# smallflyingpig/speech-to-image-translation-without-text

Hardware: AMD Instinct MI355X
Metric: StackGAN-v2 3-stage G+D train-step images/sec at 256px (higher is better)
Workload: dtype f32

## Files before the change

include/s2i_hip.h:

```cpp
#ifndef S2I_HIP_H
#define S2I_HIP_H

#include <stddef.h>
#include <stdint.h>

#ifdef __cplusplus
extern "C" {
#endif

#define S2I_ABI_VERSION 4

#define S2I_CONV_K1      0
#define S2I_CONV_K3S1    1
#define S2I_CONV_K4S2    2
#define S2I_TCONV_K4S2   3

#define S2I_CONV_1D      4

#define S2I_ACT_NONE     0
#define S2I_ACT_GLU      1
#define S2I_ACT_LRELU    2
#define S2I_ACT_TANH     3
#define S2I_ACT_RELU     4

#define S2I_DT_F32       0
#define S2I_DT_BF16      1

#define S2I_PACK_PLAIN   0
#define S2I_PACK_UPFOLD  1

const char* s2i_last_error(void);
int  s2i_version(void);
int  s2i_set_tuning(const char* key, int value);
int  s2i_get_tuning(const char* key, int* value);
int  s2i_check_device(void);

typedef struct s2i_conv_desc {
  int kind;
  int B, H, W;
  int Cx;
  int Cc;
  int N;
  int wmode;
  int flip;
  int wR;
  int ldw;
  int act;
  int stats;
  int ldy;
  int groups;
  int nosplit;
  int kw, stride, pad;
  int tile_rows;
  int in_act;
  int in_groups;
} s2i_conv_desc;

size_t s2i_conv_workspace_bytes(const s2i_conv_desc* d);
int    s2i_conv_stat_parts(const s2i_conv_desc* d);
int s2i_conv_forward(const s2i_conv_desc* d, const float* x, const float* cvec, const float* w,
                     const float* bias, float* y, float* part, void* ws, size_t ws_bytes,
                     void* stream);

int s2i_conv_forward_cls(const s2i_conv_desc* d, const float* x, const float* cvec, const float* w,
                         const float* bias, const float* cls_bias, float* y, float* part, void* ws,
                         size_t ws_bytes, void* stream);

int s2i_conv_forward_in(const s2i_conv_desc* d, const float* x_raw, const float* in_coef, const float* w, float* y,
                        float* part, void* ws, size_t ws_bytes, void* stream);

int s2i_cvec_bias_table(const float* cvec, const float* packed, int B, int Cc, int Ip, int Op, int N,
                        float* table, void* ws , size_t ws_bytes, void* stream);
size_t s2i_border_sums_workspace_bytes(int B, int H, int W, int C);
int s2i_tap_sums(const float* dy, int B, int H, int W, int C, float* tapsum, void* ws, size_t ws_bytes,
                 void* stream);
int s2i_cvec_grads(const float* cvec, const float* packed, const float* tapsum, int B, int Cc, int Ip,
                   int Op, int N, int O, int I_total, float* dc, float* dw_oihw, int accumulate,
                   void* stream);

typedef struct s2i_wgrad_desc {
  int kind;
  int B, H, W;
  int Ca;
  int Cc;
  int N;
  int ldg;
  int swap;
  int fold;
  int O, I, KH, KW;
  int accumulate;
  int i_off;
  int I_total;
  int a_act;
  int a_groups;
} s2i_wgrad_desc;

size_t s2i_wgrad_workspace_bytes(const s2i_wgrad_desc* d);
int s2i_conv_wgrad(const s2i_wgrad_desc* d, const float* a, const float* cvec, const float* g,
                   float* grad_oihw, void* ws, size_t ws_bytes, void* stream);

int s2i_conv_wgrad_in_eligible(const s2i_wgrad_desc* d);
int s2i_conv_wgrad_in(const s2i_wgrad_desc* d, const float* a_raw, const float* a_coef, const float* g,
                      float* grad_oihw, void* ws, size_t ws_bytes, void* stream);


int s2i_conv_split_eligible(const s2i_conv_desc* d);
int s2i_conv_forward_split(const s2i_conv_desc* d, const float* x, const float* cvec,
                           const unsigned short* wsplit, int planes, int np, int kp, const float* bias,
                           const float* cls_bias, float* y, float* part, void* ws, size_t ws_bytes,
                           void* stream);
size_t s2i_wgrad_workspace_bytes_split(const s2i_wgrad_desc* d, int planes);
int s2i_conv_wgrad_split(const s2i_wgrad_desc* d, int planes, const float* a, const float* cvec,
                         const float* g, float* grad_oihw, void* ws, size_t ws_bytes, void* stream);
int s2i_split_packed_weight(const float* packed, int T, int R, int C, int planes, unsigned short* out_rc,
                            unsigned short* out_cr, void* stream);


int    s2i_conv_bf16_eligible(const s2i_conv_desc* d);
size_t s2i_conv_bf16_workspace_bytes(const s2i_conv_desc* d);
int    s2i_conv_bf16_stat_parts(const s2i_conv_desc* d);
size_t s2i_conv_bf16_weight_elems(const s2i_conv_desc* d);
int    s2i_conv_bf16_weight_layout(const s2i_conv_desc* d);
int s2i_pack_conv_weight_bf16(const s2i_conv_desc* d, const float* packed, int R, int C, unsigned short* out,
                              void* stream);
typedef struct s2i_pack16_item {
  const float* P;
  unsigned short* out;
  int R, C, kind, flip, transpose, T, nphase, Nn, Npad, Kk, CK, gx, gy, block0;
} s2i_pack16_item;
int s2i_pack16_item_fill(const s2i_conv_desc* d, const float* packed, int R, int C, unsigned short* out,
                         s2i_pack16_item* item);
int s2i_pack_conv_weights_bf16_batched(const s2i_pack16_item* items_dev, int n, int total_blocks, void* stream);
int s2i_conv_forward_bf16(const s2i_conv_desc* d, const unsigned short* x, const unsigned short* w,
                          const float* cls_bias, unsigned short* y, float* part, void* ws, size_t ws_bytes,
                          void* stream);
int s2i_conv_forward_dt(const s2i_conv_desc* d, const void* x, int x_dtype, const float* cvec, const float* w,
                        const float* bias, const float* cls_bias, void* y, int y_dtype, float* part, void* ws,
                        size_t ws_bytes, void* stream);
size_t s2i_wgrad_workspace_bytes_dt(const s2i_wgrad_desc* d, int a_dtype, int g_dtype);
int s2i_conv_wgrad_dt(const s2i_wgrad_desc* d, const void* a, int a_dtype, const float* cvec, const void* g,
                      int g_dtype, float* grad_oihw, void* ws, size_t ws_bytes, void* stream);
int s2i_bn_act_forward_dt(int dtype, const void* y, long long M, int groups, int C, const float* coef4, int act,
                          const void* residual, void* out, void* stream);
int s2i_bn_act_bwd_reduce_dt(int dtype, const void* y, const void* dout, int lddout, long long M, int groups, int C,
                             const float* coef4, int act, float* part, int nparts, void* stream);
int s2i_bn_act_bwd_apply_dt(int dtype, const void* y, const void* dout, int lddout, long long M, int groups, int C,
                            const float* coef4, const float* red2, int act, void* dy, void* stream);
int s2i_act_backward_dt(int dtype, const void* out, const void* dout, int lddout, long long M, int C, int act,
                        void* dy, void* stream);
// ... 162 lines not shown
```

speech_to_image_translation_without_text_amd/_lib.py:

```python
import ctypes
import os

import torch

_HERE = os.path.dirname(os.path.abspath(__file__))
LIB_PATH = os.path.join(_HERE, "libs2i_hip.so")

CONV_K1, CONV_K3S1, CONV_K4S2, TCONV_K4S2, CONV_1D = 0, 1, 2, 3, 4
ACT_NONE, ACT_GLU, ACT_LRELU, ACT_TANH, ACT_RELU = 0, 1, 2, 3, 4
PACK_PLAIN, PACK_UPFOLD = 0, 1
DT_F32, DT_BF16 = 0, 1
POOL_MAX3S2, POOL_AVG3S1, POOL_GLOBAL = 0, 1, 2
POOL_THEN_LRN, LRN_THEN_POOL = 0, 1
LOGMEL_BFT, LOGMEL_NHWC = 0, 1
LOGMEL_TILE_FRAMES = 64
ABI_VERSION = 4

c_int, c_float, c_void_p, c_size_t, c_ll = (ctypes.c_int, ctypes.c_float, ctypes.c_void_p,
                                            ctypes.c_size_t, ctypes.c_longlong)


class ConvDesc(ctypes.Structure):
    _fields_ = [(n, c_int) for n in ("kind", "B", "H", "W", "Cx", "Cc", "N", "wmode", "flip", "wR",
                                     "ldw", "act", "stats", "ldy", "groups", "nosplit", "kw", "stride", "pad",
                                     "tile_rows", "in_act", "in_groups")]


class Conv2dDesc(ctypes.Structure):
    _fields_ = [(n, c_int) for n in ("B", "H", "W", "C", "ldx", "N", "kh", "kw", "sh", "sw", "ph", "pw", "Ho", "Wo",
                                     "ldy", "coff", "relu", "tile")]


class WgradDesc(ctypes.Structure):
    _fields_ = [(n, c_int) for n in ("kind", "B", "H", "W", "Ca", "Cc", "N", "ldg", "swap", "fold",
                                     "O", "I", "KH", "KW", "accumulate", "i_off", "I_total", "a_act", "a_groups")]


class PackItem(ctypes.Structure):
    _fields_ = [("w", c_void_p), ("packed", c_void_p)] + [(n, c_int) for n in ("O", "I", "KH", "KW", "Ip", "mode", "gx",
                                                                               "block0")]


class Pack16Item(ctypes.Structure):
    _fields_ = [("P", c_void_p), ("out", c_void_p)] + [(n, c_int) for n in (
        "R", "C", "kind", "flip", "transpose", "T", "nphase", "Nn", "Npad", "Kk", "CK", "gx", "gy", "block0")]


P = c_void_p
_SIGNATURES = {
    "s2i_last_error": (ctypes.c_char_p, []),
    "s2i_version": (c_int, []),
    "s2i_check_device": (c_int, []),
    "s2i_set_tuning": (c_int, [ctypes.c_char_p, c_int]),
    "s2i_get_tuning": (c_int, [ctypes.c_char_p, ctypes.POINTER(c_int)]),
    "s2i_conv_workspace_bytes": (c_size_t, [ctypes.POINTER(ConvDesc)]),
    "s2i_conv_stat_parts": (c_int, [ctypes.POINTER(ConvDesc)]),
    "s2i_conv_forward": (c_int, [ctypes.POINTER(ConvDesc), P, P, P, P, P, P, P, c_size_t, P]),
    "s2i_conv_forward_cls": (c_int, [ctypes.POINTER(ConvDesc), P, P, P, P, P, P, P, P, c_size_t, P]),
    "s2i_conv_forward_in": (c_int, [ctypes.POINTER(ConvDesc), P, P, P, P, P, P, c_size_t, P]),
    "s2i_conv_wgrad_in_eligible": (c_int, [ctypes.POINTER(WgradDesc)]),
    "s2i_conv_wgrad_in": (c_int, [ctypes.POINTER(WgradDesc), P, P, P, P, P, c_size_t, P]),
    "s2i_conv_split_eligible": (c_int, [ctypes.POINTER(ConvDesc)]),
    "s2i_conv_forward_split": (c_int, [ctypes.POINTER(ConvDesc), P, P, P, c_int, c_int, c_int, P, P, P, P, P, c_size_t, P]),
    "s2i_split_packed_weight": (c_int, [P, c_int, c_int, c_int, c_int, P, P, P]),
    "s2i_wgrad_workspace_bytes_split": (c_size_t, [ctypes.POINTER(WgradDesc), c_int]),
    "s2i_conv_wgrad_split": (c_int, [ctypes.POINTER(WgradDesc), c_int, P, P, P, P, P, c_size_t, P]),
    "s2i_conv_bf16_eligible": (c_int, [ctypes.POINTER(ConvDesc)]),
    "s2i_conv_bf16_workspace_bytes": (c_size_t, [ctypes.POINTER(ConvDesc)]),
    "s2i_conv_bf16_stat_parts": (c_int, [ctypes.POINTER(ConvDesc)]),
    "s2i_conv_bf16_weight_elems": (c_size_t, [ctypes.POINTER(ConvDesc)]),
    "s2i_conv_bf16_weight_layout": (c_int, [ctypes.POINTER(ConvDesc)]),
    "s2i_pack16_item_fill": (c_int, [ctypes.POINTER(ConvDesc), P, c_int, c_int, P, ctypes.POINTER(Pack16Item)]),
    "s2i_pack_conv_weights_bf16_batched": (c_int, [P, c_int, c_int, P]),
    "s2i_pack_conv_weight_bf16": (c_int, [ctypes.POINTER(ConvDesc), P, c_int, c_int, P, P]),
    "s2i_conv_forward_bf16": (c_int, [ctypes.POINTER(ConvDesc), P, P, P, P, P, P, c_size_t, P]),
    "s2i_conv_forward_dt": (c_int, [ctypes.POINTER(ConvDesc), P, c_int, P, P, P, P, P, c_int, P, P, c_size_t, P]),
    "s2i_wgrad_workspace_bytes_dt": (c_size_t, [ctypes.POINTER(WgradDesc), c_int, c_int]),
    "s2i_conv_wgrad_dt": (c_int, [ctypes.POINTER(WgradDesc), P, c_int, P, P, c_int, P, P, c_size_t, P]),
    "s2i_bn_act_forward_dt": (c_int, [c_int, P, c_ll, c_int, c_int, P, c_int, P, P, P]),
    "s2i_bn_act_bwd_reduce_dt": (c_int, [c_int, P, P, c_int, c_ll, c_int, c_int, P, c_int, P, c_int, P]),
    "s2i_bn_act_bwd_apply_dt": (c_int, [c_int, P, P, c_int, c_ll, c_int, c_int, P, P, c_int, P, P]),
    "s2i_act_backward_dt": (c_int, [c_int, P, P, c_int, c_ll, c_int, c_int, P, P]),
    "s2i_nchw_to_nhwc_dt": (c_int, [c_int, P, P, c_int, c_int, c_int, c_int, c_int, P]),
    "s2i_nhwc_to_nchw_dt": (c_int, [c_int, P, c_int, P, c_int, c_int, c_int, c_int, P]),
    "s2i_spatial_sum_dt": (c_int, [c_int, P, c_int, c_int, c_int, c_int, P, P, c_size_t, P]),
    "s2i_tap_sums_dt": (c_int, [c_int, P, c_int, c_int, c_int, c_int, P, P, c_size_t, P]),
    "s2i_cast": (c_int, [P, c_int, P, c_int, c_ll, P]),
    "s2i_cvec_bias_table": (c_int, [P, P, c_int, c_int, c_int, c_int, c_int, P, P, c_size_t, P]),
    "s2i_border_sums_workspace_bytes": (c_size_t, [c_int, c_int, c_int, c_int]),
    "s2i_tap_sums": (c_int, [P, c_int, c_int, c_int, c_int, P, P, c_size_t, P]),
    "s2i_cvec_grads": (c_int, [P, P, P, c_int, c_int, c_int, c_int, c_int, c_int, c_int, P, P, c_int, P]),
    "s2i_wgrad_workspace_bytes": (c_size_t, [ctypes.POINTER(WgradDesc)]),
    "s2i_conv_wgrad": (c_int, [ctypes.POINTER(WgradDesc), P, P, P, P, P, c_size_t, P]),
    "s2i_pack_conv_weight": (c_int, [P, P, c_int, c_int, c_int, c_int, c_int, c_int, P]),
    "s2i_pack_conv_weights_batched": (c_int, [P, c_int, c_int, c_int, P]),
    "s2i_bn_finalize": (c_int, [P, c_int, c_int, c_int, c_ll, P, P, P, P, P, c_float, c_float, P, P]),
    "s2i_bn_eval_coeffs": (c_int, [c_int, P, P, P, P, c_float, P, P]),
    "s2i_bn_act_forward": (c_int, [P, c_ll, c_int, c_int, P, c_int, P, P, P]),
    "s2i_colstats": (c_int, [P, c_ll, c_int, c_int, P, c_int, P]),
    "s2i_bn_act_bwd_reduce": (c_int, [P, P, c_int, c_ll, c_int, c_int, P, c_int, P, c_int, P]),
    "s2i_bn_bwd_finalize": (c_int, [P, c_int, c_int, c_int, c_ll, P, P, c_int, P, P]),
    "s2i_bn_act_bwd_apply": (c_int, [P, P, c_int, c_ll, c_int, c_int, P, P, c_int, P, P]),
    "s2i_act_backward": (c_int, [P, P, c_int, c_ll, c_int, c_int, P, P]),
    "s2i_glu_forward": (c_int, [P, c_ll, c_int, P, P]),
    "s2i_glu_backward": (c_int, [P, P, c_ll, c_int, P, P]),
    "s2i_nchw_to_nhwc": (c_int, [P, P, c_int, c_int, c_int, c_int, c_int, P]),
    "s2i_nhwc_to_nchw": (c_int, [P, c_int, P, c_int, c_int, c_int, c_int, P]),
    "s2i_image_to_u8": (c_int, [P, c_int, P, c_ll, P]),
    "s2i_u8_to_image": (c_int, [P, P, c_int, c_int, c_int, P]),
    "s2i_image_batch": (c_int, [P, c_ll, P, P, c_int, P, c_int, c_int, c_int, P, P, P, P, P, P]),
    "s2i_spatial_sum": (c_int, [P, c_int, c_int, c_int, c_int, P, P, c_size_t, P]),
    "s2i_spatial_sum_workspace_bytes": (c_size_t, [c_int, c_int, c_int]),
    "s2i_reparam_forward": (c_int, [P, P, c_int, c_int, P, P]),
    "s2i_reparam_backward": (c_int, [P, P, P, P, P, c_int, c_int, P, P]),
    "s2i_kl_forward": (c_int, [P, c_int, P, c_int, c_int, c_int, P, P]),
    "s2i_kl_backward": (c_int, [P, c_int, P, c_int, c_int, c_int, P, P, P, P]),
    "s2i_logit_forward": (c_int, [P, P, P, c_int, c_int, P, P]),
    "s2i_logit_backward": (c_int, [P, P, P, P, c_int, c_int, P, c_int, P, P, c_int, P]),
    "s2i_bce_forward": (c_int, [P, c_float, c_int, c_float, P, c_int, P]),
    "s2i_bce_backward": (c_int, [P, c_float, c_int, c_float, P, P, P]),
    "s2i_bce_multi_forward": (c_int, [P, P, P, c_int, c_int, c_int, P, P]),
    "s2i_bce_multi_backward": (c_int, [P, P, P, c_int, c_int, c_int, P, P, P]),
    "s2i_cal_loss": (c_int, [P, P, c_int, c_int, P, c_int, P, P]),
    "s2i_maxpool_w3s2": (c_int, [P, c_int, c_int, c_int, c_int, P, P]),
    "s2i_lstm_cell": (c_int, [P, c_int, P, P, c_int, c_int, c_int, c_int, c_int, P, P, P, c_int, P]),
    "s2i_lstm_step": (c_int, [P, c_int, P, P, P, c_int, c_int, c_int, c_int, c_int, P, P, P, P, c_int, P]),
    "s2i_time_mean": (c_int, [P, c_int, c_int, c_int, P, P]),
    "s2i_adam_step": (c_int, [P, P, P, P, c_ll, c_float, c_float, c_float, c_float, c_int, P, c_float, P]),
    "s2i_increment": (c_int, [P, P]),
    "s2i_ema_update": (c_int, [P, P, c_ll, c_float, P]),
    "s2i_scale_dev": (c_int, [P, P, c_ll, P, P]),
    "s2i_axpby": (c_int, [P, P, c_ll, c_float, c_float, P]),
    "s2i_plan_create": (c_int, [P, ctypes.POINTER(P), ctypes.POINTER(c_int)]),
    "s2i_plan_replay": (c_int, [P, P]),
    "s2i_plan_destroy": (c_int, [P]),
    "s2i_conv2d_plan": (c_int, [ctypes.POINTER(Conv2dDesc)]),
    "s2i_conv2d_weight_elems": (c_size_t, [ctypes.POINTER(Conv2dDesc)]),
    "s2i_conv2d_forward": (c_int, [ctypes.POINTER(Conv2dDesc), P, P, P, P, P]),
    "s2i_pool2d": (c_int, [c_int, P, c_int, c_int, c_int, c_int, c_int, P, c_int, c_int, P]),
    "s2i_inception_prep": (c_int, [P, c_int, c_int, c_int, c_ll, c_ll, c_ll, c_ll, P, c_int, c_int, P]),
    "s2i_softmax_rows": (c_int, [P, c_int, c_int, c_int, P, c_int, P]),
# ... 96 lines not shown
```

speech_to_image_translation_without_text_amd/csrc/s2i_common.h:

```cpp
#pragma once
#include <hip/hip_runtime.h>
#include <stdio.h>
#include <stdarg.h>
#include "../../include/s2i_hip.h"

typedef float f32x16 __attribute__((ext_vector_type(16)));
typedef float f32x4 __attribute__((ext_vector_type(4)));

void s2i_set_error(const char* fmt, ...);

#define S2I_FAIL(...)            \
  do {                           \
    s2i_set_error(__VA_ARGS__);  \
    return 1;                    \
  } while (0)

#define S2I_REQUIRE(cond, ...)   \
  do {                           \
    if (!(cond)) S2I_FAIL(__VA_ARGS__); \
  } while (0)

#define S2I_LAUNCH_CHECK(name)                                          \
  do {                                                                  \
    hipError_t e__ = hipGetLastError();                                 \
    if (e__ != hipSuccess) S2I_FAIL("%s: launch failed: %s", name, hipGetErrorString(e__)); \
  } while (0)

static inline int s2i_ilog2(int v) {
  int l = 0;
  while ((1 << l) < v) ++l;
  return l;
}
static inline bool s2i_is_pow2(int v) { return v > 0 && (v & (v - 1)) == 0; }
static inline int s2i_cdiv(long long a, long long b) { return (int)((a + b - 1) / b); }

enum {
  S2I_TUNE_FWD_BM = 0,
  S2I_TUNE_FWD_MIN_CPS,
  S2I_TUNE_B16_V2,
  S2I_TUNE_B16_PERSIST,
  S2I_TUNE_FINALIZE_THREADS,
  S2I_TUNE_B16_DBG,
  S2I_TUNE_WGRAD16_BM,
  S2I_TUNE_WGRAD_BM,
  S2I_TUNE_COUNT
};
int s2i_tune(int key, int def);
```

speech_to_image_translation_without_text_amd/csrc/s2i_conv.hip:

```cpp
#include "s2i_igemm.h"

namespace {

static int fwd_splitk(long long blocks, int nchunks, int nosplit, int min_cps) {
  int splitk = 1;
  if (blocks < 512 && nchunks >= 16 && !nosplit) {
    splitk = (int)(768 / blocks);
    if (splitk > nchunks / min_cps) splitk = nchunks / min_cps;
    if (splitk > 64) splitk = 64;
    if (splitk < 1) splitk = 1;
  }
  return splitk;
}

int plan_fwd(const s2i_conv_desc* d, FwdPlan* pl) {
  S2I_REQUIRE(d->B > 0 && d->H > 0 && d->W > 0 && d->N > 0, "conv: non-positive extent");
  S2I_REQUIRE(d->Cx >= 0 && d->Cc >= 0 && (d->Cx % 4) == 0 && (d->Cc % 4) == 0 && d->Cx + d->Cc > 0,
              "conv: channel counts must be multiples of 4 (Cx=%d Cc=%d)", d->Cx, d->Cc);
  S2I_REQUIRE(s2i_is_pow2(d->H) && s2i_is_pow2(d->W), "conv: spatial extents must be powers of two");
  pl->Ca = d->Cx + d->Cc;
  pl->nphases = 1;
  switch (d->kind) {
    case S2I_CONV_K1: pl->T = 1; pl->Ho = d->H; pl->Wo = d->W; break;
    case S2I_CONV_K3S1: pl->T = 9; pl->Ho = d->H; pl->Wo = d->W; break;
    case S2I_CONV_K4S2:
      S2I_REQUIRE(d->H >= 2 && d->W >= 2, "conv k4s2: extent < 2");
      pl->T = 16; pl->Ho = d->H / 2; pl->Wo = d->W / 2; break;
    case S2I_TCONV_K4S2: pl->T = 4; pl->Ho = d->H; pl->Wo = d->W; pl->nphases = 4; break;
    case S2I_CONV_1D:
      S2I_REQUIRE(d->kw >= 1 && d->kw <= 31 && d->stride >= 1 && d->pad >= 0, "conv1d: bad kw/stride/pad");
      S2I_REQUIRE(d->wmode == 0 && !d->flip, "conv1d: forward only");
      pl->T = d->kw; pl->Ho = d->H; pl->Wo = (d->W + 2 * d->pad - d->kw) / d->stride + 1;
      S2I_REQUIRE(pl->Wo >= 1 && s2i_is_pow2(pl->Wo), "conv1d: output width %d is not a power of two", pl->Wo);
      break;
    default: S2I_FAIL("conv: unknown kind %d", d->kind);
  }
  const long long M = (long long)d->B * pl->Ho * pl->Wo;
  S2I_REQUIRE(M * 4 < (1ll << 31), "conv: too many rows");
  pl->M = (int)M;
  pl->Mrows = M * pl->nphases;
  pl->K = pl->T * pl->Ca;
  if (d->wmode == 0) {
    S2I_REQUIRE(d->wR >= pl->Ca, "conv: wR (%d) smaller than the gathered channels (%d)", d->wR, pl->Ca);
    S2I_REQUIRE(d->ldw >= d->N && d->ldw % 4 == 0, "conv: ldw %d too small for N %d", d->ldw, d->N);
  } else {
    S2I_REQUIRE(d->wR >= d->N, "conv(T): wR (%d) < N (%d)", d->wR, d->N);
    S2I_REQUIRE(d->ldw >= pl->Ca, "conv(T): ldw (%d) < gathered channels (%d)", d->ldw, pl->Ca);
  }
  S2I_REQUIRE(d->ldy >= d->N, "conv: ldy < N");
  S2I_REQUIRE(!(d->stats && (d->act != S2I_ACT_NONE)), "conv: stats epilogue needs act NONE");
  if (d->stats && d->groups > 1) {
    S2I_REQUIRE(d->kind != S2I_TCONV_K4S2 && (M % d->groups) == 0 &&
                    (((M / d->groups) % 128) == 0 || (d->N > 64 && ((M / d->groups) % 96) == 0 && d->tile_rows != 128)),
                "conv: %lld rows do not split into %d BatchNorm groups of whole row tiles", M, d->groups);
    S2I_REQUIRE((d->N % 4) == 0, "conv: grouped statistics need N %% 4 == 0");
  }
  pl->tile = d->N > 64 ? 0 : (d->N > 32 ? 1 : 2);
  const int BN = pl->tile == 0 ? 128 : (pl->tile == 1 ? 64 : 32);
  pl->gridN = s2i_cdiv(d->N, BN);
  pl->nchunks = s2i_cdiv(pl->K, 32);
  const int forced_bm = d->tile_rows ? d->tile_rows : s2i_tune(S2I_TUNE_FWD_BM, 0);
  S2I_REQUIRE(forced_bm == 0 || forced_bm == 96 || forced_bm == 128, "conv: tile_rows must be 0, 96 or 128");
  const int min_cps = s2i_tune(S2I_TUNE_FWD_MIN_CPS, 4);
  static const int cand_bm[2] = {128, 96};
  double best = 1e300;
  int best_bm = 128, best_split = 1;
  for (int c = 0; c < 2; ++c) {
    const int bm = cand_bm[c];
    if (forced_bm ? bm != forced_bm : false) continue;
    if (bm == 96 && pl->tile != 0) continue;
    if (bm != 128 && (d->kind == S2I_CONV_1D || M < 2 * bm)) continue;
    if (d->stats && d->groups > 1 && ((M / d->groups) % bm) != 0) continue;
    const long long blocks = (long long)s2i_cdiv(M, bm) * pl->gridN * pl->nphases;
    const int sk0 = fwd_splitk(blocks, pl->nchunks, d->nosplit, min_cps);
    const int cps = s2i_cdiv(pl->nchunks, sk0), sk = s2i_cdiv(pl->nchunks, cps);
    const double rounds = (double)((blocks * sk + 767) / 768);
    const double rel = bm == 128 ? 1.0 : 0.80;
    const double slab = sk > 1 ? 3.0e-7 * sk * (double)pl->Mrows * d->N : 0.0;
    const double cost = rounds * (cps + 3.0) * rel + slab + (sk > 1 ? 2.0 : 0.0);
    if (cost < best * (bm == 128 ? 1.0 : 0.97)) { best = cost; best_bm = bm; best_split = sk; }
  }
  S2I_REQUIRE(best < 1e300 || !(d->stats && d->groups > 1 && ((M / d->groups) % 128) != 0),
              "conv: no tile height fits the %d BatchNorm groups of %lld rows", d->groups, M / (d->groups > 0 ? d->groups : 1));
  if (best == 1e300) { best_bm = 128; best_split = fwd_splitk((long long)s2i_cdiv(M, 128) * pl->gridN * pl->nphases, pl->nchunks, d->nosplit, min_cps); }
  pl->bm = best_bm;
  pl->gridM = s2i_cdiv(M, pl->bm);
  const int splitk = best_split;
  pl->cps = s2i_cdiv(pl->nchunks, splitk);
  pl->splitk = s2i_cdiv(pl->nchunks, pl->cps);
  return 0;
}

}

extern "C" size_t s2i_conv_workspace_bytes(const s2i_conv_desc* d) {
  FwdPlan pl;
  if (plan_fwd(d, &pl)) return 0;
  const size_t slab = pl.splitk > 1 ? (size_t)pl.splitk * pl.Mrows * d->N * sizeof(float) : 0;
  const size_t thin = thin_workspace_bytes(d, pl);
  return thin > slab ? thin : slab;
}

int stat_parts_for(const FwdPlan& pl, int groups) {
  if (groups < 1) groups = 1;
  if (pl.splitk > 1) {
    int ppg = s2i_cdiv(pl.Mrows / groups, 8);
    if (ppg > 512 / groups) ppg = 512 / groups;
    if (ppg < 1) ppg = 1;
    return ppg * groups;
  }
  return pl.gridM * pl.nphases;
}

extern "C" int s2i_conv_stat_parts(const s2i_conv_desc* d) {
  FwdPlan pl;
  if (plan_fwd(d, &pl)) return -1;
  return stat_parts_for(pl, d->groups);
}

static int conv_forward_impl(const s2i_conv_desc* d, const float* x, const float* cvec, const float* w,
                             const unsigned short* wsp, int planes, int np, int kp, const float* bias,
                             const float* cls_bias, float* y, float* part, void* ws, size_t ws_bytes, void* stream,
                             int x16 = 0, int y16 = 0, const float* in_coef = nullptr) {
  FwdPlan pl;
  if (plan_fwd(d, &pl)) return 1;
  S2I_REQUIRE(!cls_bias || (d->kind == S2I_CONV_K3S1 && pl.splitk == 1), "conv: class bias needs an unsplit 3x3 conv");
  S2I_REQUIRE(x != nullptr || d->Cx == 0, "conv: x is null");
  S2I_REQUIRE(d->Cc == 0 || cvec != nullptr, "conv: cvec is null but Cc > 0");
  S2I_REQUIRE((w || wsp) && y, "conv: null weight/output");
  S2I_REQUIRE(!d->stats || part, "conv: stats requested without a partial buffer");
  const size_t need = pl.splitk > 1 ? (size_t)pl.splitk * pl.Mrows * d->N * sizeof(float) : 0;
  S2I_REQUIRE(ws_bytes >= need && (need == 0 || ws), "conv: workspace too small (%zu < %zu)", ws_bytes, need);
  hipStream_t st = (hipStream_t)stream;
  IgemmP p;
  p.x = x; p.cvec = cvec; p.w = w; p.bias = bias; p.cls_bias = cls_bias; p.y = y; p.part = part; p.slab = (float*)ws;
  p.B = d->B; p.H = d->H; p.W = d->W; p.Cx = d->Cx; p.Cc = d->Cc; p.Ca = pl.Ca;
  p.Ho = pl.Ho; p.Wo = pl.Wo; p.lgWo = s2i_ilog2(pl.Wo); p.lgHoWo = s2i_ilog2(pl.Ho * pl.Wo);
  p.M = pl.M; p.N = d->N; p.K = pl.K; p.T = pl.T;
  p.kind = d->kind; p.flip = d->flip; p.act = d->act; p.stats = d->stats;
  p.splitk = pl.splitk; p.cps = pl.cps; p.nchunks = pl.nchunks;
  p.ldw = d->ldw; p.wR = d->wR; p.ldy = d->ldy; p.nparts = pl.gridM * pl.nphases;
  p.g_kw = d->kw; p.g_s = d->stride; p.g_pad = d->pad; p.wt = d->wmode != 0;
  p.Mrows = pl.Mrows;
  p.x16 = x16; p.y16 = y16;
  S2I_REQUIRE(!(wsp && (x16 || y16)), "conv(split): bf16 tensors go through s2i_conv_forward_bf16 / _dt");
  S2I_REQUIRE(!wsp || pl.bm == 128, "conv(split): the split-bf16 kernels have 128-row tiles (set tile_rows = 128)");
  p.wsp = wsp; p.wsp_np = np; p.wsp_kp = kp; p.wsp_plane = 0; p.wsp_bytes = 0;
  p.in_coef = in_coef; p.in_rows_per_group = pl.M;
  if (in_coef) {
    const int g = d->in_groups < 1 ? 1 : d->in_groups;
    S2I_REQUIRE(d->in_act == S2I_ACT_LRELU, "conv(apply-on-load): the producer's activation must be LeakyReLU (in_act=%d)", d->in_act);
    S2I_REQUIRE(!wsp && !x16 && !y16 && d->Cc == 0 && d->wmode == 0 && (pl.Ca % 32) == 0 && d->N > 4 && !bias && !cls_bias &&
                    d->kind != S2I_CONV_1D && d->kind != S2I_TCONV_K4S2,
                "conv(apply-on-load): fp32 forward of a stored tensor with 32 | Cx, no broadcast vector / bias");
    S2I_REQUIRE((pl.M % g) == 0 && (g == 1 || ((pl.M / g) % pl.bm) == 0),
                "conv(apply-on-load): %d rows do not split into %d producer groups of whole %d-row tiles", pl.M, g, pl.bm);
    p.in_rows_per_group = pl.M / g;
  }
  {
    const int r = launch_thin(d, pl, p, ws, ws_bytes, st);
    if (r >= 0) return r;
  }
  if (!wsp && d->N <= 4 && d->Cc == 0 && !d->stats && !cls_bias && (d->kind == S2I_CONV_K3S1 || d->kind == S2I_TCONV_K4S2) &&
      (pl.Ca == 16 || pl.Ca == 32 || pl.Ca == 64) && pl.M >= 4096) {
    return launch_small_n_conv(d, pl, p, st);
  }
  dim3 grid(pl.gridM, pl.gridN, pl.nphases * pl.splitk);
  const bool wt = d->wmode != 0;
  const int wtaps = d->kind == S2I_TCONV_K4S2 ? 16 : pl.T;
  const unsigned long long xb = (unsigned long long)d->B * d->H * d->W * d->Cx * (x16 ? 2ull : 4ull);
  const unsigned long long wb = (unsigned long long)wtaps * d->wR * d->ldw * 4ull;
  S2I_REQUIRE(xb < 0x7ff00000ull && wb < 0x7ff00000ull, "conv: tensor exceeds the 2 GiB buffer-addressing window");
  p.x_bytes = (unsigned)xb;
  p.c_bytes = (unsigned)((unsigned long long)d->B * d->Cc * 4ull);
  p.w_bytes = (unsigned)wb;
  const bool ca32 = (pl.Ca % 32) == 0 && (d->Cc % 32) == 0;
  if (wsp) {
    const unsigned long long pe = (unsigned long long)wtaps * np * kp;
    S2I_REQUIRE(pe * planes * 2ull < 0x7ff00000ull, "conv(split): weight planes exceed the buffer window");
    S2I_REQUIRE(kp >= pl.Ca && np >= d->N, "conv(split): weight planes %d x %d too small for N=%d K=%d", np, kp, d->N, pl.Ca);
    p.wsp_plane = (int)pe;
    p.wsp_bytes = (unsigned)(pe * planes * 2ull);
    if (launch_igemm_fwd_split(pl, p, grid, planes, st)) return 1;
  } else {
    if (launch_igemm_fwd(pl, p, grid, wt, ca32, st)) return 1;
  }
  if (pl.splitk > 1) return launch_splitk_reduce(d, pl, bias, y, part, ws, y16, stream);
  return 0;
}

extern "C" int s2i_conv_forward(const s2i_conv_desc* d, const float* x, const float* cvec, const float* w,
                                const float* bias, float* y, float* part, void* ws, size_t ws_bytes,
                                void* stream) {
  return s2i_conv_forward_cls(d, x, cvec, w, bias, nullptr, y, part, ws, ws_bytes, stream);
}

extern "C" int s2i_conv_forward_cls(const s2i_conv_desc* d, const float* x, const float* cvec, const float* w,
                                    const float* bias, const float* cls_bias, float* y, float* part, void* ws,
                                    size_t ws_bytes, void* stream) {
  S2I_REQUIRE(w != nullptr, "conv: null weight");
  return conv_forward_impl(d, x, cvec, w, nullptr, 0, 0, 0, bias, cls_bias, y, part, ws, ws_bytes, stream);
}

extern "C" int s2i_conv_forward_in(const s2i_conv_desc* d, const float* x_raw, const float* in_coef, const float* w, float* y,
                                   float* part, void* ws, size_t ws_bytes, void* stream) {
  S2I_REQUIRE(w != nullptr && in_coef != nullptr, "conv(apply-on-load): null weight / coefficient table");
  return conv_forward_impl(d, x_raw, nullptr, w, nullptr, 0, 0, 0, nullptr, nullptr, y, part, ws, ws_bytes, stream, 0, 0, in_coef);
}

extern "C" int s2i_conv_split_eligible(const s2i_conv_desc* d) {
  FwdPlan pl;
  if (plan_fwd(d, &pl)) return 0;
  const bool small_n = d->N <= 4 && d->Cc == 0 && !d->stats && (d->kind == S2I_CONV_K3S1 || d->kind == S2I_TCONV_K4S2) &&
                       (pl.Ca == 16 || pl.Ca == 32 || pl.Ca == 64) && pl.M >= 4096;
  return (pl.Ca % 32) == 0 && (d->Cc % 32) == 0 && !small_n;
}

extern "C" int s2i_conv_forward_split(const s2i_conv_desc* d, const float* x, const float* cvec,
                                      const unsigned short* wsplit, int planes, int np, int kp, const float* bias,
                                      const float* cls_bias, float* y, float* part, void* ws, size_t ws_bytes,
                                      void* stream) {
  S2I_REQUIRE(wsplit != nullptr && planes >= 1 && planes <= 3, "conv(split): need 1 to 3 bf16 planes");
  S2I_REQUIRE(np > 0 && kp > 0 && (kp % 8) == 0, "conv(split): weight rows must be multiples of 8 bf16 (kp=%d)", kp);
  S2I_REQUIRE(s2i_conv_split_eligible(d), "conv(split): layer not eligible (gathered channels must be multiples of 32)");
  return conv_forward_impl(d, x, cvec, nullptr, wsplit, planes, np, kp, bias, cls_bias, y, part, ws, ws_bytes, stream);
}

extern "C" int s2i_conv_forward_dt(const s2i_conv_desc* d, const void* x, int x_dtype, const float* cvec, const float* w,
                                   const float* bias, const float* cls_bias, void* y, int y_dtype, float* part, void* ws,
                                   size_t ws_bytes, void* stream) {
  S2I_REQUIRE(w != nullptr, "conv: null weight");
  S2I_REQUIRE((x_dtype == S2I_DT_F32 || x_dtype == S2I_DT_BF16) && (y_dtype == S2I_DT_F32 || y_dtype == S2I_DT_BF16),
              "conv: unknown dtype");
  return conv_forward_impl(d, (const float*)x, cvec, w, nullptr, 0, 0, 0, bias, cls_bias, (float*)y, part, ws, ws_bytes,
                           stream, x_dtype == S2I_DT_BF16, y_dtype == S2I_DT_BF16);
}
```

speech_to_image_translation_without_text_amd/csrc/s2i_igemm.h:

```cpp
#pragma once
#include "s2i_common.h"
#include "s2i_tile.h"

struct IgemmP {
  const float* __restrict__ x;
  const float* __restrict__ cvec;
  const float* __restrict__ w;
  const float* __restrict__ bias;
  const float* __restrict__ cls_bias;
  float* __restrict__ y;
  float* __restrict__ part;
  float* __restrict__ slab;
  int B, H, W, Cx, Cc, Ca;
  int Ho, Wo, lgWo, lgHoWo;
  int M, N, K, T;
  int kind, flip, act, stats, splitk, cps, nchunks;
  int ldw, wR, ldy, nparts;
  int g_kw, g_s, g_pad;
  int wt;
  int x16, y16;
  unsigned x_bytes, c_bytes, w_bytes;
  long long Mrows;
  const unsigned short* __restrict__ wsp;
  int wsp_np, wsp_kp, wsp_plane;
// ... 57 lines not shown
  ox = r & (p.Wo - 1);
}

template <int TM, int TN, int LDA, int LDB, int KK0 = 0, int KK1 = 16>
__device__ __forceinline__ void mma_chunk(const float* As, const float* Bs, int arow0, int bcol0,
                                          int lane, f32x16 (&acc)[TM][TN]) {
  static_assert((KK1 - KK0) % 2 == 0, "k-pairs are processed two at a time");
  const int l31 = lane & 31, lh = lane >> 5;
  const float* ap = As + lh * LDA + arow0 + l31;
  const float* bp = Bs + lh * LDB + bcol0 + l31;
  float a0[TM], b0[TN], a1[TM], b1[TN];
#pragma unroll
  for (int i = 0; i < TM; ++i) a0[i] = ap[(2 * KK0) * LDA + i * 32];
#pragma unroll
  for (int j = 0; j < TN; ++j) b0[j] = bp[(2 * KK0) * LDB + j * 32];
#pragma unroll
  for (int kk = KK0; kk < KK1; kk += 2) {
#pragma unroll
    for (int i = 0; i < TM; ++i) a1[i] = ap[(2 * (kk + 1)) * LDA + i * 32];
#pragma unroll
    for (int j = 0; j < TN; ++j) b1[j] = bp[(2 * (kk + 1)) * LDB + j * 32];
    if constexpr (TM * TN >= 4) __builtin_amdgcn_sched_barrier(0);
#pragma unroll
    for (int i = 0; i < TM; ++i)
#pragma unroll
      for (int j = 0; j < TN; ++j)
        acc[i][j] = __builtin_amdgcn_mfma_f32_32x32x2f32(a0[i], b0[j], acc[i][j], 0, 0, 0);
    if constexpr (TM * TN >= 4) __builtin_amdgcn_sched_barrier(0);
    if (kk + 2 < KK1) {
#pragma unroll
      for (int i = 0; i < TM; ++i) a0[i] = ap[(2 * (kk + 2)) * LDA + i * 32];
#pragma unroll
      for (int j = 0; j < TN; ++j) b0[j] = bp[(2 * (kk + 2)) * LDB + j * 32];
    }
    if constexpr (TM * TN >= 4) __builtin_amdgcn_sched_barrier(0);
#pragma unroll
    for (int i = 0; i < TM; ++i)
#pragma unroll
      for (int j = 0; j < TN; ++j)
        acc[i][j] = __builtin_amdgcn_mfma_f32_32x32x2f32(a1[i], b1[j], acc[i][j], 0, 0, 0);
    if constexpr (TM * TN >= 4) __builtin_amdgcn_sched_barrier(0);
  }
}

typedef unsigned int u32x4 __attribute__((ext_vector_type(4)));
#define S2I_OOB 0x7ffffff0

__device__ __forceinline__ f32x4 bload4(__amdgpu_buffer_rsrc_t r, int byte_off) {
  return __builtin_bit_cast(f32x4, __builtin_amdgcn_raw_buffer_load_b128(r, byte_off, 0, 0));
}

typedef unsigned int u32x2_t __attribute__((ext_vector_type(2)));
__device__ __forceinline__ f32x4 bload4_any(__amdgpu_buffer_rsrc_t r, int byte_off, int is16) {
  if (!is16) return bload4(r, byte_off);
  const u32x2_t v = __builtin_amdgcn_raw_buffer_load_b64(r, byte_off == S2I_OOB ? S2I_OOB : (byte_off >> 1), 0, 0);
  return f32x4{__builtin_bit_cast(float, v[0] << 16), __builtin_bit_cast(float, v[0] & 0xffff0000u),
               __builtin_bit_cast(float, v[1] << 16), __builtin_bit_cast(float, v[1] & 0xffff0000u)};
}

typedef __bf16 bf16x2 __attribute__((ext_vector_type(2)));
typedef __bf16 bf16x8 __attribute__((ext_vector_type(8)));
typedef float f32x2 __attribute__((ext_vector_type(2)));
typedef unsigned int u32x2 __attribute__((ext_vector_type(2)));

template <int NP>
__device__ __forceinline__ void split4(const f32x4 v, u32x2 (&out)[NP]) {
  f32x2 a = {v[0], v[1]}, b = {v[2], v[3]};
#pragma unroll
  for (int pl = 0; pl < NP; ++pl) {
    const unsigned pa = __builtin_bit_cast(unsigned, __builtin_convertvector(a, bf16x2));
    const unsigned pb = __builtin_bit_cast(unsigned, __builtin_convertvector(b, bf16x2));
    out[pl] = u32x2{pa, pb};
    if (pl + 1 < NP) {
      a[0] -= __builtin_bit_cast(float, pa << 16);
      a[1] -= __builtin_bit_cast(float, pa & 0xffff0000u);
      b[0] -= __builtin_bit_cast(float, pb << 16);
      b[1] -= __builtin_bit_cast(float, pb & 0xffff0000u);
    }
  }
}

struct FwdPlan {
  int T, K, Ca, Ho, Wo, M, nphases, tile, bm, gridM, gridN, nchunks, splitk, cps;
  long long Mrows;
};

struct WgPlan {
  int T, K, Cin, Ho, Wo, M, tile, gridK, gridN, nchunks, splitk, cps, small_n, rows3, bn3;
};

#pragma GCC visibility push(hidden)
int stat_parts_for(const FwdPlan& pl, int groups);
int launch_igemm_fwd(const FwdPlan& pl, const IgemmP& p, dim3 grid, bool wt, bool ca32, hipStream_t st);
int launch_igemm_fwd_split(const FwdPlan& pl, const IgemmP& p, dim3 grid, int planes, hipStream_t st);
int launch_small_n_conv(const s2i_conv_desc* d, const FwdPlan& pl, IgemmP p, hipStream_t st);
int launch_splitk_reduce(const s2i_conv_desc* d, const FwdPlan& pl, const float* bias, float* y, float* part, void* ws,
                         int y16, void* stream);
int launch_thin(const s2i_conv_desc* d, const FwdPlan& pl, IgemmP p, void* ws, size_t ws_bytes, hipStream_t st);
size_t thin_workspace_bytes(const s2i_conv_desc* d, const FwdPlan& pl);
int plan_wgrad(const s2i_wgrad_desc* d, WgPlan* pl, int planes = 0);
bool wgrad_in_ok(const s2i_wgrad_desc* d, const WgPlan& pl);
#pragma GCC visibility pop
```

speech_to_image_translation_without_text_amd/csrc/s2i_runtime.hip:

```cpp
#include "s2i_common.h"
#include <string.h>

static thread_local char g_err[512] = "";

void s2i_set_error(const char* fmt, ...) {
  va_list ap;
  va_start(ap, fmt);
  vsnprintf(g_err, sizeof(g_err), fmt, ap);
  va_end(ap);
}

extern "C" const char* s2i_last_error(void) { return g_err; }

extern "C" int s2i_version(void) { return S2I_ABI_VERSION; }

extern "C" int s2i_check_device(void) {
  int dev = 0;
  hipError_t e = hipGetDevice(&dev);
  if (e != hipSuccess) S2I_FAIL("check_device: hipGetDevice: %s", hipGetErrorString(e));
  hipDeviceProp_t prop;
  e = hipGetDeviceProperties(&prop, dev);
  if (e != hipSuccess) S2I_FAIL("check_device: hipGetDeviceProperties: %s", hipGetErrorString(e));
  if (strncmp(prop.gcnArchName, "gfx950", 6) != 0)
    S2I_FAIL("check_device: kernels are built for gfx950 only, device %d is %s", dev, prop.gcnArchName);
  return 0;
}

#include <stdlib.h>
static const char* const g_tune_names[S2I_TUNE_COUNT] = {"fwd_bm", "fwd_min_cps", "b16_v2", "b16_persist", "finalize_threads", "b16_dbg",
                                                            "wgrad16_bm", "wgrad_bm"};
static int g_tune_val[S2I_TUNE_COUNT];
static bool g_tune_set[S2I_TUNE_COUNT];

static int tune_index(const char* key, size_t len) {
  for (int i = 0; i < S2I_TUNE_COUNT; ++i)
    if (strlen(g_tune_names[i]) == len && strncmp(g_tune_names[i], key, len) == 0) return i;
  return -1;
}

namespace {
struct TuneInit {
  TuneInit() {
    const char* e = getenv("S2I_TUNE");
    while (e && *e) {
      const char* eq = strchr(e, '=');
      if (!eq) break;
      const int i = tune_index(e, (size_t)(eq - e));
      if (i >= 0) { g_tune_val[i] = atoi(eq + 1); g_tune_set[i] = true; }
      const char* c = strchr(eq, ',');
      e = c ? c + 1 : nullptr;
    }
  }
} g_tune_init;
}

int s2i_tune(int key, int def) { return g_tune_set[key] ? g_tune_val[key] : def; }

extern "C" int s2i_set_tuning(const char* key, int value) {
  const int i = key ? tune_index(key, strlen(key)) : -1;
  if (i < 0) S2I_FAIL("set_tuning: unknown key '%s'", key ? key : "(null)");
  g_tune_val[i] = value;
  g_tune_set[i] = value >= 0;
  return 0;
}

extern "C" int s2i_get_tuning(const char* key, int* value) {
  const int i = key ? tune_index(key, strlen(key)) : -1;
  if (i < 0 || !value) S2I_FAIL("get_tuning: unknown key '%s'", key ? key : "(null)");
  *value = g_tune_set[i] ? g_tune_val[i] : -1;
  return 0;
}
```

Baseline: 782.5.

## Add row-staged 3x3 conv forward kernel reusing halo rows across taps

Adds a specialized forward kernel for 3x3 stride-1 convs with 32/64 input channels, 64/128 width and N<=64. It stages whole image rows plus halo in shared memory once per vertical tap, then reuses them across the three horizontal taps instead of re-gathering im2col tiles for each tap. The planner enables it by default whenever the shape fits (f32 in/out, no split-k), and a tuning key can force the generic or row-staged path. The trade-off is larger shared memory use and lower occupancy, plus extra template instantiations.

```diff
diff --git a/include/s2i_hip.h b/include/s2i_hip.h
--- a/include/s2i_hip.h
+++ b/include/s2i_hip.h
@@ -65,6 +65,8 @@
 int s2i_conv_forward_cls(const s2i_conv_desc* d, const float* x, const float* cvec, const float* w,
                          const float* bias, const float* cls_bias, float* y, float* part, void* ws,
                          size_t ws_bytes, void* stream);
+
+int s2i_conv_fwd_variant(const s2i_conv_desc* d);
 
 int s2i_conv_forward_in(const s2i_conv_desc* d, const float* x_raw, const float* in_coef, const float* w, float* y,
                         float* part, void* ws, size_t ws_bytes, void* stream);
diff --git a/speech_to_image_translation_without_text_amd/_lib.py b/speech_to_image_translation_without_text_amd/_lib.py
--- a/speech_to_image_translation_without_text_amd/_lib.py
+++ b/speech_to_image_translation_without_text_amd/_lib.py
@@ -57,6 +57,7 @@
     "s2i_conv_stat_parts": (c_int, [ctypes.POINTER(ConvDesc)]),
     "s2i_conv_forward": (c_int, [ctypes.POINTER(ConvDesc), P, P, P, P, P, P, P, c_size_t, P]),
     "s2i_conv_forward_cls": (c_int, [ctypes.POINTER(ConvDesc), P, P, P, P, P, P, P, P, c_size_t, P]),
+    "s2i_conv_fwd_variant": (c_int, [ctypes.POINTER(ConvDesc)]),
     "s2i_conv_forward_in": (c_int, [ctypes.POINTER(ConvDesc), P, P, P, P, P, P, c_size_t, P]),
     "s2i_conv_wgrad_in_eligible": (c_int, [ctypes.POINTER(WgradDesc)]),
     "s2i_conv_wgrad_in": (c_int, [ctypes.POINTER(WgradDesc), P, P, P, P, P, c_size_t, P]),
diff --git a/speech_to_image_translation_without_text_amd/csrc/s2i_common.h b/speech_to_image_translation_without_text_amd/csrc/s2i_common.h
--- a/speech_to_image_translation_without_text_amd/csrc/s2i_common.h
+++ b/speech_to_image_translation_without_text_amd/csrc/s2i_common.h
@@ -43,6 +43,7 @@
   S2I_TUNE_B16_DBG,
   S2I_TUNE_WGRAD16_BM,
   S2I_TUNE_WGRAD_BM,
+  S2I_TUNE_FWD_K3ROWS,
   S2I_TUNE_COUNT
 };
 int s2i_tune(int key, int def);
diff --git a/speech_to_image_translation_without_text_amd/csrc/s2i_conv.hip b/speech_to_image_translation_without_text_amd/csrc/s2i_conv.hip
--- a/speech_to_image_translation_without_text_amd/csrc/s2i_conv.hip
+++ b/speech_to_image_translation_without_text_amd/csrc/s2i_conv.hip
@@ -11,6 +11,10 @@
     if (splitk < 1) splitk = 1;
   }
   return splitk;
+}
+
+static bool rows3_adopted(const s2i_conv_desc* d) {
+  return true;
 }
 
 int plan_fwd(const s2i_conv_desc* d, FwdPlan* pl) {
@@ -88,6 +92,9 @@
   const int splitk = best_split;
   pl->cps = s2i_cdiv(pl->nchunks, splitk);
   pl->splitk = s2i_cdiv(pl->nchunks, pl->cps);
+  const int k3rows = s2i_tune(S2I_TUNE_FWD_K3ROWS, 0);
+  S2I_REQUIRE(k3rows >= 0 && k3rows <= 2, "conv: fwd_k3rows must be 0 (planner), 1 (generic) or 2 (row-staged)");
+  pl->rows3 = k3rows != 1 && conv3_rows_shape_ok(d, *pl) && (k3rows == 2 || rows3_adopted(d));
   return 0;
 }
 
@@ -182,6 +189,8 @@
     p.wsp_plane = (int)pe;
     p.wsp_bytes = (unsigned)(pe * planes * 2ull);
     if (launch_igemm_fwd_split(pl, p, grid, planes, st)) return 1;
+  } else if (pl.rows3 && !x16 && !y16 && !in_coef) {
+    return launch_conv3_rows(d, pl, p, st);
   } else {
     if (launch_igemm_fwd(pl, p, grid, wt, ca32, st)) return 1;
   }
@@ -206,6 +215,12 @@
                                    float* part, void* ws, size_t ws_bytes, void* stream) {
   S2I_REQUIRE(w != nullptr && in_coef != nullptr, "conv(apply-on-load): null weight / coefficient table");
   return conv_forward_impl(d, x_raw, nullptr, w, nullptr, 0, 0, 0, nullptr, nullptr, y, part, ws, ws_bytes, stream, 0, 0, in_coef);
+}
+
+extern "C" int s2i_conv_fwd_variant(const s2i_conv_desc* d) {
+  FwdPlan pl;
+  if (plan_fwd(d, &pl)) return -1;
+  return pl.rows3 ? 2 : 1;
 }
 
 extern "C" int s2i_conv_split_eligible(const s2i_conv_desc* d) {
diff --git a/speech_to_image_translation_without_text_amd/csrc/s2i_conv_rows.hip b/speech_to_image_translation_without_text_amd/csrc/s2i_conv_rows.hip
--- /dev/null
+++ b/speech_to_image_translation_without_text_amd/csrc/s2i_conv_rows.hip
@@ -0,0 +1,175 @@
+#include "s2i_igemm.h"
+
+namespace {
+
+template <int W, int CIN, int BN, int WAVES_M, int WAVES_N, bool WT>
+__global__ __launch_bounds__(256, 3) void conv3_rows_kernel(IgemmP p) {
+  constexpr int BM = 128, R = BM / W;
+  constexpr int TM = BM / (WAVES_M * 32), TN = BN / (WAVES_N * 32);
+  constexpr int TB = CIN == 32 ? 3 : 1;
+  constexpr int NPIX = R * (W + 2);
+  constexpr int LD = NPIX | 1;
+  constexpr int LDB = WT ? BN + 1 : BN;
+  constexpr int CQ = CIN / 4;
+  constexpr int AELEMS = ((NPIX + 3) / 4) * 4 * CQ, APASS = (AELEMS + 255) / 256;
+  constexpr int KB = TB * CIN;
+  constexpr int BROWS = 1024 / BN, BPASS = WT ? (BN / 32) * (KB / 32) : KB / BROWS;
+  static_assert(R * W == BM && (W % 32) == 0 && (CIN % 32) == 0 && (3 % TB) == 0, "tile geometry");
+  static_assert((TM * 32) <= W, "the rows of a wave lie in one image row");
+  __shared__ __attribute__((aligned(16))) float smem[KB * LDB + CIN * LD];
+  float* Bs = smem;
+  float* As = smem + KB * LDB;
+
+  const int tid = threadIdx.x, lane = tid & 63, wave = tid >> 6;
+  const int wm = wave / WAVES_N, wn = wave % WAVES_N;
+  const int G = gridDim.x, L = blockIdx.x;
+  const int bx = (G & 7) == 0 ? (L & 7) * (G >> 3) + (L >> 3) : L;
+  const int m0 = bx * BM, n0 = 0;
+  const int img = m0 >> p.lgHoWo;
+  const int oy0 = (m0 & ((1 << p.lgHoWo) - 1)) >> p.lgWo;
+
+  const __amdgpu_buffer_rsrc_t rx = __builtin_amdgcn_make_buffer_rsrc((void*)p.x, 0, p.x_bytes, 0x00020000);
+  const __amdgpu_buffer_rsrc_t rw = __builtin_amdgcn_make_buffer_rsrc((void*)p.w, 0, p.w_bytes, 0x00020000);
+
+  int agx[APASS], alds[APASS], arow[APASS];
+#pragma unroll
+  for (int q = 0; q < APASS; ++q) {
+    const int e = tid + q * 256;
+    const int rest = e >> 5;
+    const int cq = (rest % (CQ / 8)) * 8 + (e & 7);
+    const int pidx = (rest / (CQ / 8)) * 4 + ((e >> 3) & 3);
+    const int r = R == 1 ? 0 : pidx / (W + 2), ix = pidx - r * (W + 2) - 1;
+    const bool have = pidx < NPIX;
+    arow[q] = r;
+    alds[q] = have ? cq * 4 * LD + pidx : -1;
+    agx[q] = (have && ix >= 0 && ix < W) ? (((img * p.H + oy0 + r - 1) * W + ix) * CIN + cq * 4) * 4 : S2I_OOB;
+  }
+  const int kq = tid & 7, mrow = tid >> 3;
+  const int bcol4 = tid % (BN / 4), brow = tid / (BN / 4);
+  int wconst[BN / 32];
+#pragma unroll
+  for (int j = 0; j < BN / 32; ++j) {
+    if constexpr (WT) {
+      const int n = n0 + mrow + 32 * j;
+      wconst[j] = n < p.N ? (n * p.ldw + kq * 4) * 4 : S2I_OOB;
+    } else {
+      wconst[j] = n0 + bcol4 * 4 < p.ldw ? (n0 + bcol4 * 4) * 4 : S2I_OOB;
+    }
+  }
+
+  f32x4 ra[APASS], rb[BPASS];
+  auto fetch_a = [&](int dy) {
+#pragma unroll
+    for (int q = 0; q < APASS; ++q) {
+      const int iy = oy0 + arow[q] + dy - 1;
+      ra[q] = bload4(rx, (agx[q] != S2I_OOB && iy >= 0 && iy < p.H) ? agx[q] + dy * W * CIN * 4 : S2I_OOB);
+    }
+  };
+  auto fetch_b = [&](int t0) {
+    if constexpr (WT) {
+#pragma unroll
+      for (int q = 0; q < BPASS; ++q) {
+        const int ch = q / (BN / 32), j = q % (BN / 32);
+        const int tw = tap_weight(S2I_CONV_K3S1, p.flip, 9, t0 + ch / (CIN / 32), 0, 0);
+        const int c0 = (ch % (CIN / 32)) * 32;
+        rb[q] = bload4(rw, wconst[j] == S2I_OOB ? S2I_OOB : (tw * p.wR * p.ldw + c0) * 4 + wconst[j]);
+      }
+    } else {
+#pragma unroll
+      for (int q = 0; q < BPASS; ++q) {
+        const int kr = brow + q * BROWS;
+        const int tw = tap_weight(S2I_CONV_K3S1, p.flip, 9, t0 + kr / CIN, 0, 0);
+        rb[q] = bload4(rw, wconst[0] == S2I_OOB ? S2I_OOB : (tw * p.wR + kr % CIN) * p.ldw * 4 + wconst[0]);
+      }
+    }
+  };
+  auto store_a = [&]() {
+#pragma unroll
+    for (int q = 0; q < APASS; ++q)
+      if (alds[q] >= 0) {
+#pragma unroll
+        for (int j = 0; j < 4; ++j) As[alds[q] + j * LD] = ra[q][j];
+      }
+  };
+  auto store_b = [&]() {
+    if constexpr (WT) {
+#pragma unroll
+      for (int q = 0; q < BPASS; ++q) {
+        const int ch = q / (BN / 32), j = q % (BN / 32);
+#pragma unroll
+        for (int jj = 0; jj < 4; ++jj) Bs[(ch * 32 + kq * 4 + jj) * LDB + mrow + 32 * j] = rb[q][jj];
+      }
+    } else {
+#pragma unroll
+      for (int q = 0; q < BPASS; ++q) *reinterpret_cast<f32x4*>(Bs + (brow + q * BROWS) * LDB + bcol4 * 4) = rb[q];
+    }
+  };
+
+  f32x16 acc[TM][TN];
+  zero_acc(acc);
+  const int wrow = wm * TM * 32;
+  const float* ap = As + (wrow / W) * (W + 2) + (wrow % W);
+
+  fetch_a(0);
+  fetch_b(0);
+#pragma unroll 1
+  for (int t0 = 0; t0 < 9; t0 += TB) {
+    const int dx0 = t0 % 3;
+    if (dx0 == 0) store_a();
+    store_b();
+    __syncthreads();
+    if (t0 + TB < 9) {
+      fetch_b(t0 + TB);
+      if ((t0 + TB) % 3 == 0) fetch_a((t0 + TB) / 3);
+    }
+#pragma unroll 1
+    for (int dxl = 0; dxl < TB; ++dxl)
+#pragma unroll
+      for (int cc = 0; cc < CIN / 32; ++cc)
+        mma_chunk<TM, TN, LD, LDB>(ap + cc * 32 * LD + dx0 + dxl, Bs + (dxl * CIN + cc * 32) * LDB, 0, wn * TN * 32, lane, acc);
+    __syncthreads();
+  }
+
+  if (p.cls_bias)
+    add_class_bias<TM, TN>(p.cls_bias, p.N, p.Ho, p.Wo, acc, lane, wm, wn, n0, [&](int r, int& b, int& oy, int& ox) {
+      row_pixel(p, m0 + r, b, oy, ox);
+      return true;
+    });
+  store_tile<TM, TN>(p.y, p.ldy, p.N, false, p.bias, p.act, 0, acc, lane, wm, wn, n0, [&](int r, long long& row) {
+    row = m0 + r;
+    return true;
+  });
+  if (p.stats) tile_col_stats<TM, TN, WAVES_M, BN>(p.part, p.nparts, p.N, smem, acc, tid, lane, wm, wn, n0, bx);
+}
+
+template <int W, int CIN>
+void launch_rows(const IgemmP& p, dim3 grid, bool wide, bool wt, hipStream_t st) {
+  if (wide) {
+    if (wt) hipLaunchKernelGGL((conv3_rows_kernel<W, CIN, 64, 2, 2, true>), grid, dim3(256), 0, st, p);
+    else hipLaunchKernelGGL((conv3_rows_kernel<W, CIN, 64, 2, 2, false>), grid, dim3(256), 0, st, p);
+  } else {
+    if (wt) hipLaunchKernelGGL((conv3_rows_kernel<W, CIN, 32, 4, 1, true>), grid, dim3(256), 0, st, p);
+    else hipLaunchKernelGGL((conv3_rows_kernel<W, CIN, 32, 4, 1, false>), grid, dim3(256), 0, st, p);
+  }
+}
+
+}
+
+bool conv3_rows_shape_ok(const s2i_conv_desc* d, const FwdPlan& pl) {
+  return d->kind == S2I_CONV_K3S1 && d->Cc == 0 && (d->Cx == 32 || d->Cx == 64) && (d->W == 64 || d->W == 128) && d->H >= 2 &&
+         d->N > 4 && d->N <= 64 && pl.bm == 128 && pl.splitk == 1 && (pl.M % 128) == 0 && pl.gridN == 1;
+}
+
+int launch_conv3_rows(const s2i_conv_desc* d, const FwdPlan& pl, const IgemmP& p, hipStream_t st) {
+  const dim3 grid(pl.gridM);
+  const bool wide = pl.tile == 1, wt = d->wmode != 0;
+  if (d->W == 128) {
+    if (d->Cx == 32) launch_rows<128, 32>(p, grid, wide, wt, st);
+    else launch_rows<128, 64>(p, grid, wide, wt, st);
+  } else {
+    if (d->Cx == 32) launch_rows<64, 32>(p, grid, wide, wt, st);
+    else launch_rows<64, 64>(p, grid, wide, wt, st);
+  }
+  S2I_LAUNCH_CHECK("conv3_rows");
+  return 0;
+}
diff --git a/speech_to_image_translation_without_text_amd/csrc/s2i_igemm.h b/speech_to_image_translation_without_text_amd/csrc/s2i_igemm.h
--- a/speech_to_image_translation_without_text_amd/csrc/s2i_igemm.h
+++ b/speech_to_image_translation_without_text_amd/csrc/s2i_igemm.h
@@ -163,6 +163,7 @@
 
 struct FwdPlan {
   int T, K, Ca, Ho, Wo, M, nphases, tile, bm, gridM, gridN, nchunks, splitk, cps;
+  int rows3;
   long long Mrows;
 };
 
@@ -177,6 +178,8 @@
 int launch_small_n_conv(const s2i_conv_desc* d, const FwdPlan& pl, IgemmP p, hipStream_t st);
 int launch_splitk_reduce(const s2i_conv_desc* d, const FwdPlan& pl, const float* bias, float* y, float* part, void* ws,
                          int y16, void* stream);
+bool conv3_rows_shape_ok(const s2i_conv_desc* d, const FwdPlan& pl);
+int launch_conv3_rows(const s2i_conv_desc* d, const FwdPlan& pl, const IgemmP& p, hipStream_t st);
 int launch_thin(const s2i_conv_desc* d, const FwdPlan& pl, IgemmP p, void* ws, size_t ws_bytes, hipStream_t st);
 size_t thin_workspace_bytes(const s2i_conv_desc* d, const FwdPlan& pl);
 int plan_wgrad(const s2i_wgrad_desc* d, WgPlan* pl, int planes = 0);
diff --git a/speech_to_image_translation_without_text_amd/csrc/s2i_runtime.hip b/speech_to_image_translation_without_text_amd/csrc/s2i_runtime.hip
--- a/speech_to_image_translation_without_text_amd/csrc/s2i_runtime.hip
+++ b/speech_to_image_translation_without_text_amd/csrc/s2i_runtime.hip
@@ -28,7 +28,7 @@
 
 #include <stdlib.h>
 static const char* const g_tune_names[S2I_TUNE_COUNT] = {"fwd_bm", "fwd_min_cps", "b16_v2", "b16_persist", "finalize_threads", "b16_dbg",
-                                                            "wgrad16_bm", "wgrad_bm"};
+                                                            "wgrad16_bm", "wgrad_bm", "fwd_k3rows"};
 static int g_tune_val[S2I_TUNE_COUNT];
 static bool g_tune_set[S2I_TUNE_COUNT];
 
```

New measurement: 785.5 (median of 6 runs). No clear change (+0.4%).
